# KikeM/romtime

Hardware: AMD Instinct MI355X
Metric: snapshot-DoF/s for POD build (higher is better)
Workload: dtype f64

## Files before the change

romtime_amd/csrc/gemm_panel.h:

```cpp
#pragma once
#include "common.h"

typedef double d4 __attribute__((ext_vector_type(4)));
typedef double d2 __attribute__((ext_vector_type(2)));

namespace rtk {

constexpr int KB = 16;
constexpr int NTHREADS = 256;
constexpr int KSTRIDE = KB + 2;

struct GemmParams {
  const double* A; long a_ks, a_ms;
  const double* B; long b_ks, b_ns;
  double* C; long c_rs, c_cs, c_split_stride;
  long K, M, Nn, k_per_split;
  int tiles_m, tiles_n, ntiles, splits, symmetric, vecA, vecB;
  double c_alpha, c_beta;
};

template <int BT, bool KC, int NTHR = NTHREADS>
struct Panel {
  static constexpr int NL = (KB * BT / 2) / NTHR;
  static constexpr int SM = BT + 16;
  static constexpr int LDS = KC ? BT * KSTRIDE : KB * SM;

  static __device__ __forceinline__ void load(d2 (&regs)[NL], const double* __restrict__ P, long ks, long ms,
                                              long k0, long kend, long m0, long Mext, int vec, int tid) {
#pragma unroll
    for (int j = 0; j < NL; ++j) {
      const int q = tid + NTHR * j;
      int kk, i;
      const double* p;
      bool v0, v1;
      if (!KC) {
        kk = q / (BT / 2);
        i = (q % (BT / 2)) * 2;
        const long k = k0 + kk, m = m0 + i;
        p = P + k * ks + m * ms;
        v0 = (k < kend) && (m < Mext);
        v1 = (k < kend) && (m + 1 < Mext);
        if (vec && v1) {
          regs[j] = *reinterpret_cast<const d2*>(p);
        } else {
          regs[j].x = v0 ? p[0] : 0.0;
          regs[j].y = v1 ? p[ms] : 0.0;
        }
      } else {
        i = q / (KB / 2);
        kk = (q % (KB / 2)) * 2;
        const long k = k0 + kk, m = m0 + i;
        p = P + m * ms + k * ks;
        v0 = (m < Mext) && (k < kend);
        v1 = (m < Mext) && (k + 1 < kend);
        if (vec && v1) {
          regs[j] = *reinterpret_cast<const d2*>(p);
        } else {
          regs[j].x = v0 ? p[0] : 0.0;
          regs[j].y = v1 ? p[ks] : 0.0;
        }
      }
    }
  }

  static __device__ __forceinline__ void load_full(d2 (&regs)[NL], const double* __restrict__ P, long ks, long ms,
                                                   long k0, long m0, int tid) {
#pragma unroll
    for (int j = 0; j < NL; ++j) {
      const int q = tid + NTHR * j;
      if (!KC) {
        const int kk = q / (BT / 2), i = (q % (BT / 2)) * 2;
        regs[j] = *reinterpret_cast<const d2*>(P + (k0 + kk) * ks + (m0 + i));
      } else {
        const int i = q / (KB / 2), kk = (q % (KB / 2)) * 2;
        regs[j] = *reinterpret_cast<const d2*>(P + (m0 + i) * ms + (k0 + kk));
      }
    }
  }

  static __device__ __forceinline__ unsigned lane_offset(long ks, long ms, int tid) {
    return KC ? (unsigned)(((long)(tid / (KB / 2)) * ms + (tid % (KB / 2)) * 2) * 8)
              : (unsigned)(((long)(tid / (BT / 2)) * ks + (tid % (BT / 2)) * 2) * 8);
  }
  static __device__ __forceinline__ long load_step(long ks, long ms) {
    return KC ? (long)(NTHR / (KB / 2)) * ms * 8 : (long)(NTHR / (BT / 2)) * ks * 8;
  }
  static __device__ __forceinline__ void load_full_u(d2 (&regs)[NL], const char* __restrict__ base, unsigned voff,
                                                     long rows_step_bytes) {
#pragma unroll
    for (int j = 0; j < NL; ++j) regs[j] = *reinterpret_cast<const d2*>(base + j * rows_step_bytes + voff);
  }

  static __device__ __forceinline__ void store(const d2 (&regs)[NL], double* s, int tid) {
#pragma unroll
    for (int j = 0; j < NL; ++j) {
      const int q = tid + NTHR * j;
      if (!KC) {
        const int kk = q / (BT / 2), i = (q % (BT / 2)) * 2;
        *reinterpret_cast<d2*>(&s[kk * SM + i]) = regs[j];
      } else {
        const int i = q / (KB / 2), kk = (q % (KB / 2)) * 2;
        *reinterpret_cast<d2*>(&s[i * KSTRIDE + kk]) = regs[j];
      }
    }
  }

  static __device__ __forceinline__ double frag(const double* s, int mloc, int k4, int l15, int l4) {
    return KC ? s[(mloc + l15) * KSTRIDE + k4 * 4 + l4] : s[(k4 * 4 + l4) * SM + mloc + l15];
  }
};

}
```

romtime_amd/csrc/gram_mfma.hip:

```cpp
#include <algorithm>
#include <type_traits>

#include "gemm_panel.h"

using namespace rtk;

namespace {

constexpr int BT = 128;
constexpr int GT = 512;
constexpr int MAX_SLOTS = 64;
constexpr int MAX_TILES = 36;
typedef unsigned u2 __attribute__((ext_vector_type(2)));
constexpr unsigned long long PACE_ONE = 1ull << 40;
constexpr int PACE_DROP = 6;

struct GramParams {
  const double* X;
  long ks, ms;
  long K, n, kx;
  long last0;
  double* slab;
  int nslots, tiles1, vec;
  long* counters;
  unsigned long long* pace;
  int pace_every, pace_slack, pace_naps;
  unsigned char slot_tm[MAX_SLOTS], slot_tn[MAX_SLOTS], slot_q[MAX_SLOTS], slot_S[MAX_SLOTS];
};

struct GramSegs {
  unsigned char tm[MAX_SLOTS], tn[MAX_SLOTS], q[MAX_SLOTS], S[MAX_SLOTS];
  unsigned short slab[MAX_SLOTS];
};

__device__ const unsigned char kDiagTi[8][5] = {{0, 0, 0, 0, 0}, {0, 0, 0, 1, 1}, {1, 1, 1, 1, 1}, {2, 2, 2, 2, 2}, {2, 3, 3, 3, 255}, {3, 3, 4, 4, 255}, {4, 4, 5, 5, 255}, {5, 6, 6, 7, 255}};
__device__ const unsigned char kDiagTj[8][5] = {{0, 1, 2, 3, 4}, {5, 6, 7, 1, 2}, {3, 4, 5, 6, 7}, {2, 3, 4, 5, 6}, {7, 3, 4, 5, 0}, {6, 7, 4, 5, 0}, {6, 7, 5, 6, 0}, {7, 6, 7, 7, 0}};

template <bool KC, bool DIAG>
__device__ __forceinline__ void gram_segment(const GramParams& p, double* smem, int x, int tm, int tn, int q0, int S,
                                             double* out) {
  using P = Panel<BT, KC, GT>;
  double* sA0 = smem;
  double* sA1 = smem + P::LDS;
  double* sB0 = smem + 2 * P::LDS;
  double* sB1 = smem + 3 * P::LDS;

  int tid = threadIdx.x;
  asm volatile("" : "+v"(tid));
  const long m0 = (tm == p.tiles1 - 1) ? p.last0 : (long)tm * BT, n0 = (tn == p.tiles1 - 1) ? p.last0 : (long)tn * BT;
  const long kend_x = ((long)x * p.kx + p.kx < p.K) ? (long)x * p.kx + p.kx : p.K;
  const int nst_x = (kend_x > (long)x * p.kx) ? (int)((kend_x - (long)x * p.kx + KB - 1) / KB) : 0;
  const long kbeg = (long)x * p.kx;
  const long kend = kend_x;
  const int nstages = (nst_x > q0) ? (nst_x - q0 + S - 1) / S : 0;

  const int lane = tid & 63, wid = tid >> 6;
  const int wm = wid >> 2, wn = wid & 3;
  const int l15 = lane & 15, l4 = lane >> 4;

  unsigned long long* pace = p.pace ? p.pace + 16 * x : nullptr;
  int pacer = (pace && __builtin_amdgcn_readfirstlane(wid) == 0 && nstages > 0) ? 1 : 0;
  int pace_pos = 0, pace_cnt = 0;
  if (pacer && lane == 0) __hip_atomic_fetch_add(pace, PACE_ONE, __ATOMIC_RELAXED, __HIP_MEMORY_SCOPE_AGENT);

  constexpr int NACC = DIAG ? 5 : 8;
  d4 acc[NACC];
#pragma unroll
  for (int i = 0; i < NACC; ++i) acc[i] = d4{0.0, 0.0, 0.0, 0.0};
  int dti[5], dtj[5];
  bool dval[5];
  {
    const int w = __builtin_amdgcn_readfirstlane(wid);
#pragma unroll
    for (int q = 0; q < 5; ++q) {
      dval[q] = kDiagTi[w][q] != 255;
      dti[q] = dval[q] ? 16 * kDiagTi[w][q] : 0;
      dtj[q] = 16 * kDiagTj[w][q];
    }
  }

  d2 ra[P::NL], rb[DIAG ? 1 : P::NL];
  const bool interior = p.vec && (m0 + BT <= p.n) && (n0 + BT <= p.n);
  if (nstages > 0) {
    const long k0 = kbeg + (long)q0 * KB;
    P::load(ra, p.X, p.ks, p.ms, k0, kend, m0, p.n, p.vec, tid);
    if constexpr (!DIAG) P::load(rb, p.X, p.ks, p.ms, k0, kend, n0, p.n, p.vec, tid);
    P::store(ra, sA0, tid);
    if constexpr (!DIAG) P::store(rb, sB0, tid);
  }
  __syncthreads();

  const long k1 = kbeg + (long)(q0 + S) * KB;
  const char* gA = reinterpret_cast<const char*>(p.X + k1 * p.ks + m0 * p.ms);
  const char* gB = reinterpret_cast<const char*>(p.X + k1 * p.ks + n0 * p.ms);
  const unsigned voff = P::lane_offset(p.ks, p.ms, tid);
  const long rows_step = P::load_step(p.ks, p.ms), stage_step = (long)S * KB * p.ks * 8;

  int n_full = nstages;
  if (nstages > 0 && kbeg + (long)(q0 + (nstages - 1) * S) * KB + KB > kend) n_full = nstages - 1;
  if (!interior) n_full = 0;

  auto compute = [&](const double* cA, const double* cB) {
    if constexpr (DIAG) {
#pragma unroll
      for (int k4 = 0; k4 < KB / 4; ++k4) {
#pragma unroll
        for (int q = 0; q < 5; ++q) {
          if (!dval[q]) continue;
          const double a = P::frag(cA, dti[q], k4, l15, l4);
          const double b = P::frag(cA, dtj[q], k4, l15, l4);
          acc[q] = __builtin_amdgcn_mfma_f64_16x16x4f64(a, b, acc[q], 0, 0, 0);
        }
      }
    } else {
#pragma unroll
      for (int k4 = 0; k4 < KB / 4; ++k4) {
        double a[4], b[2];
#pragma unroll
        for (int i = 0; i < 4; ++i) a[i] = P::frag(cA, wm * 64 + i * 16, k4, l15, l4);
#pragma unroll
        for (int j = 0; j < 2; ++j) b[j] = P::frag(cB, wn * 32 + j * 16, k4, l15, l4);
#pragma unroll
        for (int i = 0; i < 4; ++i)
#pragma unroll
          for (int j = 0; j < 2; ++j)
            acc[i * 2 + j] = __builtin_amdgcn_mfma_f64_16x16x4f64(a[i], b[j], acc[i * 2 + j], 0, 0, 0);
      }
    }
  };

  int st = 0;
  {
    auto fast_stage = [&](auto parity) {
      constexpr int PAR = decltype(parity)::value;
      P::load_full_u(ra, gA, voff, rows_step);
      if constexpr (!DIAG) P::load_full_u(rb, gB, voff, rows_step);
      const bool check = pacer && ++pace_cnt == p.pace_every;
      unsigned long long before = 0;
      if (check) {
        pace_cnt = 0;
        const int adv = S * p.pace_every;
        if (lane == 0) before = __hip_atomic_fetch_add(pace, (unsigned long long)adv, __ATOMIC_RELAXED, __HIP_MEMORY_SCOPE_AGENT);
        pace_pos += adv;
      }
      __builtin_amdgcn_s_setprio(1);
      compute(PAR ? sA1 : sA0, PAR ? sB1 : sB0);
      __builtin_amdgcn_s_setprio(0);
      gA += stage_step;
      gB += stage_step;
      P::store(ra, PAR ? sA0 : sA1, tid);
      if constexpr (!DIAG) P::store(rb, PAR ? sB0 : sB1, tid);
      if (check) {
        unsigned lo = __builtin_amdgcn_readfirstlane((unsigned)before), hi = __builtin_amdgcn_readfirstlane((unsigned)(before >> 32));
        unsigned long long word = (((unsigned long long)hi << 32) | lo) + (unsigned long long)(S * p.pace_every);
#pragma unroll 1
        for (int nap = 0;; ++nap) {
          const long long total = (long long)(word & (PACE_ONE - 1)), members = (long long)(word >> 40);
          const long long lead = (long long)pace_pos * members - total;
          if (lead < -(long long)PACE_DROP * S * members) {
            if (lane == 0)
              __hip_atomic_fetch_add(pace, 0ull - (PACE_ONE + (unsigned long long)pace_pos), __ATOMIC_RELAXED,
                                     __HIP_MEMORY_SCOPE_AGENT);
            pacer = 0;
            break;
          }
          if (lead <= (long long)p.pace_slack * S * members || nap >= p.pace_naps) break;
          __builtin_amdgcn_s_sleep(16);
          u2 v;
          asm volatile("s_load_dwordx2 %0, %1, 0x0 glc\n\ts_waitcnt lgkmcnt(0)" : "=s"(v) : "s"(pace) : "memory");
          word = ((unsigned long long)v.y << 32) | v.x;
        }
      }
      __syncthreads();
    };
    for (; st + 2 < n_full; st += 2) {
      fast_stage(std::integral_constant<int, 0>{});
      fast_stage(std::integral_constant<int, 1>{});
    }
  }
  for (; st < nstages; ++st) {
    const double* cA = (st & 1) ? sA1 : sA0;
    const double* cB = (st & 1) ? sB1 : sB0;
    const bool more = st + 1 < nstages;
    if (more) {
      const long k0 = kbeg + (long)(q0 + (st + 1) * S) * KB;
      if (st + 1 < n_full) {
        P::load_full(ra, p.X, p.ks, p.ms, k0, m0, tid);
        if constexpr (!DIAG) P::load_full(rb, p.X, p.ks, p.ms, k0, n0, tid);
      } else {
        P::load(ra, p.X, p.ks, p.ms, k0, kend, m0, p.n, p.vec, tid);
        if constexpr (!DIAG) P::load(rb, p.X, p.ks, p.ms, k0, kend, n0, p.n, p.vec, tid);
      }
    }
    __builtin_amdgcn_s_setprio(1);
    compute(cA, cB);
    __builtin_amdgcn_s_setprio(0);
    if (more) {
      P::store(ra, (st & 1) ? sA0 : sA1, tid);
      if constexpr (!DIAG) P::store(rb, (st & 1) ? sB0 : sB1, tid);
    }
    __syncthreads();
  }

  if constexpr (DIAG) {
#pragma unroll
    for (int q = 0; q < 5; ++q)
#pragma unroll
      for (int r = 0; r < 4; ++r)
        if (dval[q]) out[(dti[q] + l4 + 4 * r) * BT + dtj[q] + l15] = acc[q][r];
  } else {
#pragma unroll
    for (int i = 0; i < 4; ++i)
#pragma unroll
      for (int j = 0; j < 2; ++j)
#pragma unroll
        for (int r = 0; r < 4; ++r)
          out[(wm * 64 + i * 16 + l4 + 4 * r) * BT + wn * 32 + j * 16 + l15] = acc[i * 2 + j][r];
  }
}

__device__ __forceinline__ void gram_check_xcd(const GramParams& p, int x) {
  if (threadIdx.x == 0 && (int)(__builtin_amdgcn_s_getreg((31 << 11) | 20) & 15u) != x)
    atomicAdd(reinterpret_cast<unsigned long long*>(&p.counters[RT_CNT_GRAM_OFF_XCD]), 1ull);
}

template <bool KC, bool DIAG>
__global__ __launch_bounds__(GT, 4) void gram128_kernel(const GramParams p) {
  extern __shared__ __attribute__((aligned(16))) double smem[];
  const int x = blockIdx.x & 7, slot = blockIdx.x >> 3;
  gram_check_xcd(p, x);
  const int tm = __builtin_amdgcn_readfirstlane((int)p.slot_tm[slot]), tn = __builtin_amdgcn_readfirstlane((int)p.slot_tn[slot]),
            q0 = __builtin_amdgcn_readfirstlane((int)p.slot_q[slot]), S = __builtin_amdgcn_readfirstlane((int)p.slot_S[slot]);
  gram_segment<KC, DIAG>(p, smem, x, tm, tn, q0, S, p.slab + ((long)x * p.nslots + slot) * (BT * BT));
}

template <bool KC>
__global__ __launch_bounds__(GT, 4) void gram128_merged_kernel(const GramParams p, const GramSegs g) {
  extern __shared__ __attribute__((aligned(16))) double smem[];
  const int x = blockIdx.x & 7, slot = blockIdx.x >> 3;
  gram_check_xcd(p, x);
  const int S = __builtin_amdgcn_readfirstlane((int)g.S[slot]);
  if (S == 0) return;
  const int tm = __builtin_amdgcn_readfirstlane((int)g.tm[slot]), tn = __builtin_amdgcn_readfirstlane((int)g.tn[slot]),
            q0 = __builtin_amdgcn_readfirstlane((int)g.q[slot]), slab = __builtin_amdgcn_readfirstlane((int)g.slab[slot]);
  double* out = p.slab + ((long)x * p.nslots + slab) * (BT * BT);
  if (tm == tn)
    gram_segment<KC, true>(p, smem, x, tm, tn, q0, S, out);
  else
    gram_segment<KC, false>(p, smem, x, tm, tn, q0, S, out);
}

struct GramReduceParams {
  const double* slab_off;
  const double* slab_diag;
  double* G;
  long n, last0;
  int nslots_off, nslots_diag, tiles1;
  unsigned char first[MAX_TILES], count[MAX_TILES];
  unsigned long long* pace;
};

__global__ void gram_reduce_kernel(const GramReduceParams p) {
  const long idx = (long)blockIdx.x * blockDim.x + threadIdx.x;
  if (p.pace && idx < 256) p.pace[idx] = 0ull;
  if (idx >= p.n * p.n) return;
  const long i = idx / p.n, j = idx % p.n;
  if (i > j) return;
  const int tm = (int)(i / BT), tn = (int)(j / BT);
  const int t = tm * p.tiles1 - tm * (tm - 1) / 2 + (tn - tm);
  const long off = (i - (tm == p.tiles1 - 1 ? p.last0 : (long)tm * BT)) * BT + (j - (tn == p.tiles1 - 1 ? p.last0 : (long)tn * BT));
  const double* slab = (tm == tn) ? p.slab_diag : p.slab_off;
  const int nslots = (tm == tn) ? p.nslots_diag : p.nslots_off;
  const int cnt = p.count[t];
  const double* base = slab + (long)p.first[t] * (BT * BT) + off;
  double sum = 0.0;
  for (int x = 0; x < 8; ++x) {
    const double* src = base + (long)x * nslots * (BT * BT);
#pragma unroll 4
    for (int q = 0; q < cnt; ++q) sum += src[(long)q * (BT * BT)];
  }
  p.G[idx] = sum;
  if (i != j) p.G[j * p.n + i] = sum;
}

template <bool KC, bool DIAG>
int launch_gram(rt_ctx* ctx, const GramParams& p, int grid) {
  const size_t lds = sizeof(double) * (DIAG ? 2 : 4) * Panel<BT, KC, GT>::LDS;
  RT_TRY(rt_func_lds(ctx, reinterpret_cast<const void*>(&gram128_kernel<KC, DIAG>), (int)lds));
  hipLaunchKernelGGL((gram128_kernel<KC, DIAG>), dim3(grid), dim3(GT), lds, ctx->stream, p);
  RT_HIP_CHECK(ctx, hipGetLastError());
  return RT_OK;
}

constexpr double GRAM_RHO = 0.60;

struct GramPace {
  int every, slack, naps;
};
constexpr GramPace PACE_TWO_LAUNCHES{2, 2, 8}, PACE_ONE_LAUNCH{2, 1, 8};

double gram_uniform_ab(int P, int n_off, int n_d, double rho, int cap, int* a_out, int* b_out) {
  double best = 1e30;
  int best_slots = 0;
  *a_out = *b_out = 0;
  for (int a = 1; a <= cap && n_off * a + n_d <= P; ++a)
    for (int b = 1; b <= cap && n_off * a + n_d * b <= P; ++b) {
      const double T = (1.0 / a > rho / b) ? 1.0 / a : rho / b;
      const int used = n_off * a + n_d * b;
      if (T < best - 1e-12 || (T < best + 1e-12 && used < best_slots)) { best = T; *a_out = a; *b_out = b; best_slots = used; }
    }
  return *a_out ? best : 0.0;
}

int gram_plan(int tiles1, int s_off, int s_diag, GramSegs& g, unsigned char* first, unsigned char* count) {
  g = GramSegs{};
  int slot = 0;
  for (int diag = 0; diag < 2; ++diag) {
    const int S = diag ? s_diag : s_off;
    int t = 0;
    for (int a = 0; a < tiles1; ++a)
      for (int b = a; b < tiles1; ++b, ++t) {
        if ((a == b) != (diag == 1)) continue;
        first[t] = (unsigned char)slot;
        count[t] = (unsigned char)S;
        for (int q = 0; q < S; ++q, ++slot) {
          g.tm[slot] = (unsigned char)a; g.tn[slot] = (unsigned char)b;
          g.q[slot] = (unsigned char)q; g.S[slot] = (unsigned char)S;
          g.slab[slot] = (unsigned short)slot;
        }
      }
  }
  return slot;
}

struct GramChoice {
  int form, a, b, s_off, s_diag, slots;
};
GramChoice gram_choose(int num_cus, long K, long n) {
  const int slots_max = 2 * num_cus / 8;
  GramChoice c{0, 0, 0, 0, 0, slots_max};
  const int tiles1 = (int)((n + BT - 1) / BT), ntiles = tiles1 * (tiles1 + 1) / 2, n_off = ntiles - tiles1;
  if (n < 97 || ntiles > MAX_TILES || n_off > slots_max || slots_max > MAX_SLOTS || K < 8L * 64 * KB) return c;
  const long kx = ((K + 7) / 8 + KB - 1) / KB * KB;
  const int cap = (int)(kx / KB / 48);
  if (cap < 1) return c;
  c.s_off = n_off ? std::min(slots_max / n_off, cap) : 0;
  c.s_diag = std::min(slots_max / tiles1, cap);
  if (n_off >= 1) {
    const double t_uni = gram_uniform_ab(slots_max, n_off, tiles1, GRAM_RHO, cap, &c.a, &c.b);
    const double t_two = (c.s_off >= 1 && c.s_diag >= 1) ? 1.0 / c.s_off + GRAM_RHO / c.s_diag : 0.0;
    if (t_uni > 0.0 && t_two > 0.0 && t_uni <= 1.05 * t_two && n_off * c.a + tiles1 * c.b >= 16 && !(tiles1 == 2 && c.a >= cap)) {
      c.form = 2;
      return c;
    }
  }
  const int busiest = n_off ? n_off * c.s_off : tiles1 * c.s_diag;
  c.form = (busiest >= 16) ? 1 : 0;
  return c;
}

template <bool KC>
int launch_gram_merged(rt_ctx* ctx, const GramParams& p, const GramSegs& g, int grid) {
  constexpr size_t lds = sizeof(double) * 4 * Panel<BT, KC, GT>::LDS;
  RT_TRY(rt_func_lds(ctx, reinterpret_cast<const void*>(&gram128_merged_kernel<KC>), (int)lds));
  hipLaunchKernelGGL((gram128_merged_kernel<KC>), dim3(grid), dim3(GT), lds, ctx->stream, p, g);
  RT_HIP_CHECK(ctx, hipGetLastError());
  return RT_OK;
}

}

int rt_gram128(rt_ctx* ctx, const double* X, int64_t ks, int64_t ms, int64_t K, int64_t n, double* G) {
  if (!(ks == 1 || ms == 1)) return RT_ERR_UNSUPPORTED;
  const GramChoice c = gram_choose(ctx->num_cus, (long)K, (long)n);
  if (c.form == 0) return RT_ERR_UNSUPPORTED;
  const bool one_launch = c.form == 2;
  const bool kc = (ks == 1) && (ms != 1);
  const int tiles1 = (int)((n + BT - 1) / BT), n_off = tiles1 * (tiles1 - 1) / 2;

  GramParams p;
  p.X = X; p.ks = ks; p.ms = ms; p.K = K; p.n = n;
  p.kx = ((K + 7) / 8 + KB - 1) / KB * KB;
  p.tiles1 = tiles1;
  const long other = kc ? ms : ks;
  p.vec = ((((uintptr_t)X) & 15) == 0 && (other % 2 == 0)) ? 1 : 0;
  p.last0 = (long)(tiles1 - 1) * BT;
  if (n % BT != 0 && n >= BT && p.vec && (kc || n % 2 == 0)) p.last0 = n - BT;
  if ((!kc && (long)ks * 8 * 8 >= (1L << 31)) || (kc && (long)ms * 64 * 8 >= (1L << 31))) p.vec = 0;
  p.counters = ctx->dev_counters;
  p.pace = nullptr;
  const GramPace pace = one_launch ? PACE_ONE_LAUNCH : PACE_TWO_LAUNCHES;
  p.pace_every = pace.every; p.pace_slack = pace.slack; p.pace_naps = pace.naps;
  if (ctx->gram_pace_on) {
    if (!ctx->gram_pace) {
      RT_HIP_CHECK(ctx, hipMalloc(reinterpret_cast<void**>(&ctx->gram_pace), sizeof(unsigned long long) * 256));
      RT_HIP_CHECK(ctx, hipMemsetAsync(ctx->gram_pace, 0, sizeof(unsigned long long) * 256, ctx->stream));
    }
    p.pace = ctx->gram_pace;
  }

  GramSegs g;
  GramReduceParams rp;
  int nslots_off, nslots_diag;
  if (one_launch) {
    nslots_off = nslots_diag = gram_plan(tiles1, c.a, c.b, g, rp.first, rp.count);
  } else {
    nslots_off = c.s_off * n_off;
    nslots_diag = c.s_diag * tiles1;
  }
  void* slab = nullptr;
  int rc = rt_scratch(ctx, sizeof(double) * BT * BT * 8 * (size_t)(one_launch ? nslots_off : nslots_off + nslots_diag), &slab);
  if (rc != RT_OK) return rc;
  double* slab_off = static_cast<double*>(slab);
  double* slab_diag = one_launch ? slab_off : slab_off + (size_t)8 * nslots_off * BT * BT;
  rp.slab_off = slab_off; rp.slab_diag = slab_diag; rp.G = G; rp.n = n; rp.last0 = p.last0;
  rp.nslots_off = nslots_off; rp.nslots_diag = nslots_diag; rp.tiles1 = tiles1; rp.pace = ctx->gram_pace;

  if (ctx->profile) {
    if (!ctx->ev0) {
      RT_HIP_CHECK(ctx, hipEventCreate(&ctx->ev0));
      RT_HIP_CHECK(ctx, hipEventCreate(&ctx->ev1));
    }
    if (!ctx->gev0) {
      RT_HIP_CHECK(ctx, hipEventCreate(&ctx->gev0));
      RT_HIP_CHECK(ctx, hipEventCreate(&ctx->gev1));
    }
    RT_HIP_CHECK(ctx, hipEventRecord(ctx->ev0, ctx->stream));
    RT_HIP_CHECK(ctx, hipEventRecord(ctx->gev0, ctx->stream));
  }
  if (one_launch) {
    p.slab = slab_off; p.nslots = nslots_off;
    rc = kc ? launch_gram_merged<true>(ctx, p, g, 8 * c.slots) : launch_gram_merged<false>(ctx, p, g, 8 * c.slots);
    if (rc != RT_OK) return rc;
  } else {
    if (n_off) {
      int slot = 0, t = 0;
      for (int a = 0; a < tiles1; ++a)
        for (int b = a; b < tiles1; ++b, ++t) {
          if (a == b) continue;
          rp.first[t] = (unsigned char)slot; rp.count[t] = (unsigned char)c.s_off;
          for (int q = 0; q < c.s_off; ++q, ++slot) {
            p.slot_tm[slot] = (unsigned char)a; p.slot_tn[slot] = (unsigned char)b;
            p.slot_q[slot] = (unsigned char)q; p.slot_S[slot] = (unsigned char)c.s_off;
          }
        }
      p.slab = slab_off; p.nslots = nslots_off;
      rc = kc ? launch_gram<true, false>(ctx, p, 8 * nslots_off) : launch_gram<false, false>(ctx, p, 8 * nslots_off);
      if (rc != RT_OK) return rc;
    }
    {
      int slot = 0, t = 0;
      for (int a = 0; a < tiles1; ++a)
        for (int b = a; b < tiles1; ++b, ++t) {
          if (a != b) continue;
          rp.first[t] = (unsigned char)slot; rp.count[t] = (unsigned char)c.s_diag;
          for (int q = 0; q < c.s_diag; ++q, ++slot) {
            p.slot_tm[slot] = (unsigned char)a; p.slot_tn[slot] = (unsigned char)a;
            p.slot_q[slot] = (unsigned char)q; p.slot_S[slot] = (unsigned char)c.s_diag;
          }
        }
      p.slab = slab_diag; p.nslots = nslots_diag;
      p.pace = nullptr;
      rc = kc ? launch_gram<true, true>(ctx, p, 8 * nslots_diag) : launch_gram<false, true>(ctx, p, 8 * nslots_diag);
      if (rc != RT_OK) return rc;
    }
  }
  if (ctx->profile) {
    RT_HIP_CHECK(ctx, hipEventRecord(ctx->ev1, ctx->stream));
    RT_HIP_CHECK(ctx, hipEventRecord(ctx->gev1, ctx->stream));
    ctx->ev_valid = true;
    ctx->gev_valid = true;
  }
  ctx->last_grid = one_launch ? 8 * c.slots : 8 * (nslots_off + nslots_diag);
  ctx->last_splits = 8 * (one_launch ? c.a : c.s_off);
  ctx->last_tile = 128 * 1000 + 128;
  const long total = n * n;
  hipLaunchKernelGGL(gram_reduce_kernel, dim3((unsigned)((total + 255) / 256)), dim3(256), 0, ctx->stream, rp);
  RT_HIP_CHECK(ctx, hipGetLastError());
  return RT_OK;
}

extern "C" int rt_gram_plan_info(int num_cus, int64_t n_rows, int64_t n_cols, int* out) {
  if (!out || num_cus < 8 || n_rows < 1 || n_cols < 1) return RT_ERR_ARG;
  const GramChoice c = gram_choose(num_cus, (long)n_rows, (long)n_cols);
  out[0] = c.form; out[1] = c.a; out[2] = c.b; out[3] = c.s_off; out[4] = c.s_diag;
  return RT_OK;
}
```

Baseline: 92.20 billion.

## Rebalance diagonal Gram tile work with 4x4 MFMA upper-triangle blocks

Replaces the per-wave assignment of 16x16 sub-tiles for diagonal Gram tiles with a new scheme. Each wave now computes three or four off-diagonal 16x16 blocks. The 16x16 diagonal blocks are covered only in their upper triangle, using 4x4x4 f64 MFMAs on rotated fragments. This cuts redundant lower-triangle work on diagonal blocks and evens out MFMA counts across waves. The cost is more complex indexing, extra LDS reads for the rotated fragments, and a scattered write of the diagonal results.

```diff
diff --git a/romtime_amd/csrc/gemm_panel.h b/romtime_amd/csrc/gemm_panel.h
--- a/romtime_amd/csrc/gemm_panel.h
+++ b/romtime_amd/csrc/gemm_panel.h
@@ -105,6 +105,8 @@
     }
   }
 
+  static __device__ __forceinline__ constexpr int at(int c, int kk) { return KC ? c * KSTRIDE + kk : kk * SM + c; }
+
   static __device__ __forceinline__ double frag(const double* s, int mloc, int k4, int l15, int l4) {
     return KC ? s[(mloc + l15) * KSTRIDE + k4 * 4 + l4] : s[(k4 * 4 + l4) * SM + mloc + l15];
   }
diff --git a/romtime_amd/csrc/gram_mfma.hip b/romtime_amd/csrc/gram_mfma.hip
--- a/romtime_amd/csrc/gram_mfma.hip
+++ b/romtime_amd/csrc/gram_mfma.hip
@@ -33,8 +33,8 @@
   unsigned short slab[MAX_SLOTS];
 };
 
-__device__ const unsigned char kDiagTi[8][5] = {{0, 0, 0, 0, 0}, {0, 0, 0, 1, 1}, {1, 1, 1, 1, 1}, {2, 2, 2, 2, 2}, {2, 3, 3, 3, 255}, {3, 3, 4, 4, 255}, {4, 4, 5, 5, 255}, {5, 6, 6, 7, 255}};
-__device__ const unsigned char kDiagTj[8][5] = {{0, 1, 2, 3, 4}, {5, 6, 7, 1, 2}, {3, 4, 5, 6, 7}, {2, 3, 4, 5, 6}, {7, 3, 4, 5, 0}, {6, 7, 4, 5, 0}, {6, 7, 5, 6, 0}, {7, 6, 7, 7, 0}};
+__device__ const unsigned char kDiagV[8][4] = {{0, 1, 3, 4}, {1, 5, 7, 6}, {2, 3, 6, 7}, {3, 4, 7, 5},
+                                               {0, 2, 5, 0}, {0, 6, 7, 0}, {1, 2, 4, 0}, {4, 5, 6, 0}};
 
 template <bool KC, bool DIAG>
 __device__ __forceinline__ void gram_segment(const GramParams& p, double* smem, int x, int tm, int tn, int q0, int S,
@@ -63,20 +63,25 @@
   int pace_pos = 0, pace_cnt = 0;
   if (pacer && lane == 0) __hip_atomic_fetch_add(pace, PACE_ONE, __ATOMIC_RELAXED, __HIP_MEMORY_SCOPE_AGENT);
 
-  constexpr int NACC = DIAG ? 5 : 8;
+  constexpr int NACC = DIAG ? 4 : 8;
   d4 acc[NACC];
 #pragma unroll
   for (int i = 0; i < NACC; ++i) acc[i] = d4{0.0, 0.0, 0.0, 0.0};
-  int dti[5], dtj[5];
-  bool dval[5];
-  {
+  double dacc[3] = {0.0, 0.0, 0.0};
+  int dv[4] = {0, 0, 0, 0}, dd = 0;
+  int ofr[4] = {0, 0, 0, 0}, orot[2] = {0, 0};
+  bool paw = false;
+  if constexpr (DIAG) {
     const int w = __builtin_amdgcn_readfirstlane(wid);
-#pragma unroll
-    for (int q = 0; q < 5; ++q) {
-      dval[q] = kDiagTi[w][q] != 255;
-      dti[q] = dval[q] ? 16 * kDiagTi[w][q] : 0;
-      dtj[q] = 16 * kDiagTj[w][q];
-    }
+    paw = w < 4;
+#pragma unroll
+    for (int q = 0; q < 4; ++q) {
+      dv[q] = kDiagV[w][q];
+      ofr[q] = P::at(16 * dv[q] + l15, l4);
+    }
+    dd = paw ? dv[0] : dv[2];
+#pragma unroll
+    for (int s = 1; s <= 2; ++s) orot[s - 1] = P::at(16 * dd + 4 * (((lane >> 2) + s) & 3) + (lane & 3), l4);
   }
 
   d2 ra[P::NL], rb[DIAG ? 1 : P::NL];
@@ -104,12 +109,24 @@
     if constexpr (DIAG) {
 #pragma unroll
       for (int k4 = 0; k4 < KB / 4; ++k4) {
-#pragma unroll
-        for (int q = 0; q < 5; ++q) {
-          if (!dval[q]) continue;
-          const double a = P::frag(cA, dti[q], k4, l15, l4);
-          const double b = P::frag(cA, dtj[q], k4, l15, l4);
-          acc[q] = __builtin_amdgcn_mfma_f64_16x16x4f64(a, b, acc[q], 0, 0, 0);
+        const int ok = P::at(0, 4 * k4);
+        const double f0 = cA[ofr[0] + ok], f1 = cA[ofr[1] + ok], f2 = cA[ofr[2] + ok];
+        const double r1 = cA[orot[0] + ok], r2 = cA[orot[1] + ok];
+        double f3 = 0.0;
+        if (paw) f3 = cA[ofr[3] + ok];
+        acc[0] = __builtin_amdgcn_mfma_f64_16x16x4f64(f0, f1, acc[0], 0, 0, 0);
+        acc[1] = __builtin_amdgcn_mfma_f64_16x16x4f64(f0, f2, acc[1], 0, 0, 0);
+        acc[2] = __builtin_amdgcn_mfma_f64_16x16x4f64(f1, f2, acc[2], 0, 0, 0);
+        auto triangle = [&](double f) {
+          dacc[0] = __builtin_amdgcn_mfma_f64_4x4x4f64(f, f, dacc[0], 0, 0, 0);
+          dacc[1] = __builtin_amdgcn_mfma_f64_4x4x4f64(f, r1, dacc[1], 0, 0, 0);
+          dacc[2] = __builtin_amdgcn_mfma_f64_4x4x4f64(f, r2, dacc[2], 0, 0, 0);
+        };
+        if (paw) {
+          triangle(f0);
+          acc[3] = __builtin_amdgcn_mfma_f64_16x16x4f64(f0, f3, acc[3], 0, 0, 0);
+        } else {
+          triangle(f2);
         }
       }
     } else {
@@ -203,11 +220,19 @@
   }
 
   if constexpr (DIAG) {
-#pragma unroll
-    for (int q = 0; q < 5; ++q)
-#pragma unroll
-      for (int r = 0; r < 4; ++r)
-        if (dval[q]) out[(dti[q] + l4 + 4 * r) * BT + dtj[q] + l15] = acc[q][r];
+    auto put = [&](int u, int v, const d4& a) {
+#pragma unroll
+      for (int r = 0; r < 4; ++r) out[(16 * u + l4 + 4 * r) * BT + 16 * v + l15] = a[r];
+    };
+    put(dv[0], dv[1], acc[0]);
+    put(dv[0], dv[2], acc[1]);
+    put(dv[1], dv[2], acc[2]);
+    if (paw) put(dv[0], dv[3], acc[3]);
+    const int I = (lane >> 2) & 3, row = 16 * dd + 4 * I + l4, c0 = 16 * dd + (lane & 3);
+    out[row * BT + c0 + 4 * I] = dacc[0];
+    if (I < 3) out[row * BT + c0 + 4 * (I + 1)] = dacc[1];
+    else out[c0 * BT + row] = dacc[1];
+    if (I < 2) out[row * BT + c0 + 4 * (I + 2)] = dacc[2];
   } else {
 #pragma unroll
     for (int i = 0; i < 4; ++i)
```

After: 92.97 billion, median of 6. Within noise of the previous version (+0.8%).
